# hku-mars/GS-SDF

Hardware: NVIDIA H100
Metric: train_steps_per_s (higher is better)
Workload: dtype f32

## Files before the change

gs-sdf_b200/csrc/sh.cu:

```cuda
#include "common.cuh"

namespace gssdf {

template <int DEG>
__device__ __forceinline__ void sh_bases(float x, float y, float z, float *b) {
    b[0] = 0.2820947917738781f;
    if (DEG < 1) return;
    b[1] = -0.48860251190292f * y; b[2] = 0.48860251190292f * z; b[3] = -0.48860251190292f * x;
    if (DEG < 2) return;
    const float z2 = z * z;
    const float fTmp0B = -1.092548430592079f * z;
    const float fC1 = x * x - y * y, fS1 = 2.f * x * y;
    b[6] = 0.9461746957575601f * z2 - 0.3153915652525201f;
    b[7] = fTmp0B * x; b[5] = fTmp0B * y;
    b[8] = 0.5462742152960395f * fC1; b[4] = 0.5462742152960395f * fS1;
    if (DEG < 3) return;
    const float fTmp0C = -2.285228997322329f * z2 + 0.4570457994644658f;
    const float fTmp1B = 1.445305721320277f * z;
    const float fC2 = x * fC1 - y * fS1, fS2 = x * fS1 + y * fC1;
    b[12] = z * (1.865881662950577f * z2 - 1.119528997770346f);
    b[13] = fTmp0C * x; b[11] = fTmp0C * y;
    b[14] = fTmp1B * fC1; b[10] = fTmp1B * fS1;
    b[15] = -0.5900435899266435f * fC2; b[9] = -0.5900435899266435f * fS2;
    if (DEG < 4) return;
// ... 45 lines not shown
        const float fTmp0D = z * (-4.683325804901025f * z2 + 2.007139630671868f);
        const float fTmp0D_z = 3.f * -4.683325804901025f * z2 + 2.007139630671868f;
        const float fTmp1C = 3.31161143515146f * z2 - 0.47308734787878f;
        const float fTmp1C_z = 2.f * 3.31161143515146f * z;
        const float fTmp2B = -1.770130769779931f * z, fTmp2B_z = -1.770130769779931f;
        const float fC3_x = fC2 + x * fC2_x - y * fS2_x, fC3_y = x * fC2_y - fS2 - y * fS2_y;
        const float fS3_x = fS2 + y * fC2_x + x * fS2_x, fS3_y = x * fS2_y + fC2 + y * fC2_y;
        const float pSH20_z = 1.984313483298443f * (pSH12 + z * pSH12_z) - 1.006230589874905f * pSH6_z;
        vx += 0.6258357354491763f * fS3_x * w[16] + 0.6258357354491763f * fC3_x * w[24] + fTmp2B * fS2_x * w[17] +
              fTmp2B * fC2_x * w[23] + fTmp1C * fS1_x * w[18] + fTmp1C * fC1_x * w[22] + fTmp0D * w[21];
        vy += 0.6258357354491763f * fS3_y * w[16] + 0.6258357354491763f * fC3_y * w[24] + fTmp2B * fS2_y * w[17] +
              fTmp2B * fC2_y * w[23] + fTmp1C * fS1_y * w[18] + fTmp1C * fC1_y * w[22] + fTmp0D * w[19];
        vz += pSH20_z * w[20] + fTmp0D_z * x * w[21] + fTmp0D_z * y * w[19] + fTmp1C_z * fC1 * w[22] +
              fTmp1C_z * fS1 * w[18] + fTmp2B_z * fC2 * w[23] + fTmp2B_z * fS2 * w[17];
    }
}

__device__ __forceinline__ void cam_centre(const float *viewmats, int cid, float c[3]) {
    const float *v = viewmats + 16 * cid;
#pragma unroll
    for (int r = 0; r < 3; ++r) c[r] = -(v[0 + r] * v[3] + v[4 + r] * v[7] + v[8 + r] * v[11]);
}

template <int DEG>
__global__ void __launch_bounds__(256) view_colors_fwd_kernel(const gssdf_view_colors_fwd_args a) {
    constexpr int KU = (DEG + 1) * (DEG + 1);
    const int nnz = a.counts->nnz;
    const int i = blockIdx.x * blockDim.x + threadIdx.x;
    if (i >= nnz) return;
    const int64_t g = a.gaussian_ids[i];
    const int2 rad = reinterpret_cast<const int2 *>(a.radii)[i];
    float out[3] = {0.f, 0.f, 0.f};
    if (rad.x > 0 && rad.y > 0) {
        float cc[3];
        cam_centre(a.viewmats, (int)a.camera_ids[i], cc);
        float dx = a.means[3 * g] - cc[0], dy = a.means[3 * g + 1] - cc[1], dz = a.means[3 * g + 2] - cc[2];
        if (a.mean_offsets) { dx += a.mean_offsets[3 * g]; dy += a.mean_offsets[3 * g + 1]; dz += a.mean_offsets[3 * g + 2]; }
        float x = 0.f, y = 0.f, z = 0.f;
        if (DEG >= 1) {
            const float inorm = rsqrtf(dx * dx + dy * dy + dz * dz);
            x = dx * inorm; y = dy * inorm; z = dz * inorm;
        }
        float b[KU];
        sh_bases<DEG>(x, y, z, b);
        const float *co = a.sh_rest ? a.sh + (size_t)g * 3 : a.sh + (size_t)g * a.K * 3;
        const float *cr = a.sh_rest ? a.sh_rest + (size_t)g * (a.K - 1) * 3 - 3 : co;
#pragma unroll
        for (int k = 0; k < KU; ++k) {
            const float *c = k == 0 ? co : cr + 3 * k;
            out[0] += b[k] * __ldg(c);
            out[1] += b[k] * __ldg(c + 1);
            out[2] += b[k] * __ldg(c + 2);
        }
#pragma unroll
        for (int c = 0; c < 3; ++c) out[c] = fmaxf(out[c] + 0.5f, 0.f);
    }
    a.colors[3 * (int64_t)i] = out[0];
    a.colors[3 * (int64_t)i + 1] = out[1];
    a.colors[3 * (int64_t)i + 2] = out[2];
}

template <int DEG>
__global__ void __launch_bounds__(256) view_colors_bwd_kernel(const gssdf_view_colors_bwd_args a) {
    constexpr int KU = (DEG + 1) * (DEG + 1);
    const int nnz = a.counts->nnz;
    const int i = blockIdx.x * blockDim.x + threadIdx.x;
    if (i >= nnz) return;
    const int2 rad = reinterpret_cast<const int2 *>(a.radii)[i];
    if (!(rad.x > 0 && rad.y > 0)) return;
    const int64_t g = a.gaussian_ids[i];
    float vc[3];
#pragma unroll
    for (int c = 0; c < 3; ++c) {
        const float col = a.colors[3 * (int64_t)i + c];
        vc[c] = col > 0.f ? a.v_colors[3 * (int64_t)i + c] : 0.f;
    }
    float cc[3];
    cam_centre(a.viewmats, (int)a.camera_ids[i], cc);
    float dx = a.means[3 * g] - cc[0], dy = a.means[3 * g + 1] - cc[1], dz = a.means[3 * g + 2] - cc[2];
    if (a.mean_offsets) { dx += a.mean_offsets[3 * g]; dy += a.mean_offsets[3 * g + 1]; dz += a.mean_offsets[3 * g + 2]; }
    float x = 0.f, y = 0.f, z = 0.f, inorm = 1.f;
    if (DEG >= 1) {
// ... 7 lines not shown
    float *vsr = split ? a.v_sh_rest + (size_t)g * (a.K - 1) * 3 - 3 : vsh;
    const float *co = split ? a.sh + (size_t)g * 3 : a.sh + (size_t)g * a.K * 3;
    const float *cr = split ? a.sh_rest + (size_t)g * (a.K - 1) * 3 - 3 : co;
    float w[KU];
#pragma unroll
    for (int k = 0; k < KU; ++k) {
        float *v = k == 0 ? vsh : vsr + 3 * k;
        const float *c = k == 0 ? co : cr + 3 * k;
        atomicAdd(v, b[k] * vc[0]);
        atomicAdd(v + 1, b[k] * vc[1]);
        atomicAdd(v + 2, b[k] * vc[2]);
        w[k] = __ldg(c) * vc[0] + __ldg(c + 1) * vc[1] + __ldg(c + 2) * vc[2];
    }
    if (DEG >= 1 && a.v_means) {
        float vx, vy, vz;
        sh_bases_vjp<DEG>(x, y, z, w, vx, vy, vz);
        const float d = vx * x + vy * y + vz * z;
        atomicAdd(a.v_means + 3 * g, (vx - d * x) * inorm);
        atomicAdd(a.v_means + 3 * g + 1, (vy - d * y) * inorm);
        atomicAdd(a.v_means + 3 * g + 2, (vz - d * z) * inorm);
    }
}

}

using namespace gssdf;

extern "C" int gssdf_view_colors_fwd(const gssdf_view_colors_fwd_args *a, gssdf_stream_t stream) {
    GSSDF_REQUIRE(a != nullptr, GSSDF_EINVAL, "view_colors_fwd: null args");
    if (a->cap == 0 || a->N == 0) return GSSDF_OK;
    GSSDF_REQUIRE(a->sh_degree >= 0 && a->sh_degree <= 4, GSSDF_EINVAL, "view_colors_fwd: sh_degree %d not in [0,4]", a->sh_degree);
    GSSDF_REQUIRE((a->sh_degree + 1) * (a->sh_degree + 1) <= a->K, GSSDF_EINVAL,
                  "view_colors_fwd: Invalid coeffs shape: (deg+1)^2=%d > K=%d", (a->sh_degree + 1) * (a->sh_degree + 1), a->K);
    GSSDF_REQUIRE(a->viewmats && a->means && a->sh && a->counts && a->camera_ids && a->gaussian_ids && a->radii && a->colors,
                  GSSDF_EINVAL, "view_colors_fwd: null pointer");
    cudaStream_t st = (cudaStream_t)stream;
    const int grid = cdiv(a->cap, 256);
    switch (a->sh_degree) {
        case 0: view_colors_fwd_kernel<0><<<grid, 256, 0, st>>>(*a); break;
        case 1: view_colors_fwd_kernel<1><<<grid, 256, 0, st>>>(*a); break;
        case 2: view_colors_fwd_kernel<2><<<grid, 256, 0, st>>>(*a); break;
        case 3: view_colors_fwd_kernel<3><<<grid, 256, 0, st>>>(*a); break;
        default: view_colors_fwd_kernel<4><<<grid, 256, 0, st>>>(*a); break;
    }
    GSSDF_LAUNCH_OK("view_colors_fwd_kernel");
    return GSSDF_OK;
}

extern "C" int gssdf_view_colors_bwd(const gssdf_view_colors_bwd_args *a, gssdf_stream_t stream) {
    GSSDF_REQUIRE(a != nullptr, GSSDF_EINVAL, "view_colors_bwd: null args");
    if (a->cap == 0 || a->N == 0) return GSSDF_OK;
    GSSDF_REQUIRE(a->sh_degree >= 0 && a->sh_degree <= 4, GSSDF_EINVAL, "view_colors_bwd: sh_degree %d not in [0,4]", a->sh_degree);
    GSSDF_REQUIRE((a->sh_degree + 1) * (a->sh_degree + 1) <= a->K, GSSDF_EINVAL, "view_colors_bwd: Invalid coeffs shape");
    GSSDF_REQUIRE(a->viewmats && a->means && a->sh && a->counts && a->camera_ids && a->gaussian_ids && a->radii &&
                      a->colors && a->v_colors && a->v_sh,
                  GSSDF_EINVAL, "view_colors_bwd: null pointer");
    GSSDF_REQUIRE(!a->sh_rest || (a->v_sh_rest && a->K >= 2), GSSDF_EINVAL, "view_colors_bwd: sh_rest needs v_sh_rest and K >= 2");
    cudaStream_t st = (cudaStream_t)stream;
    const int grid = cdiv(a->cap, 256);
    switch (a->sh_degree) {
        case 0: view_colors_bwd_kernel<0><<<grid, 256, 0, st>>>(*a); break;
        case 1: view_colors_bwd_kernel<1><<<grid, 256, 0, st>>>(*a); break;
        case 2: view_colors_bwd_kernel<2><<<grid, 256, 0, st>>>(*a); break;
        case 3: view_colors_bwd_kernel<3><<<grid, 256, 0, st>>>(*a); break;
        default: view_colors_bwd_kernel<4><<<grid, 256, 0, st>>>(*a); break;
    }
    GSSDF_LAUNCH_OK("view_colors_bwd_kernel");
    return GSSDF_OK;
}
```

gs-sdf_b200/gssdf_b200/cabi.py:

```python
import math

import torch

from . import _lib
from ._lib import check, lib, make_args

COUNTS_INTS = 8
NNZ, N_ISECTS, NNZ_OVERFLOW, ISECT_OVERFLOW, MAX_TILE = 0, 1, 2, 3, 4


def _stream():
    return torch.cuda.current_stream().cuda_stream


def _req(t, dtype, name):
    if t is None:
        return None
    if not t.is_cuda:
        raise ValueError(f"gssdf_b200: {name} must be a CUDA tensor")
    if not t.is_contiguous():
        raise ValueError(f"gssdf_b200: {name} must be contiguous")
    if t.dtype != dtype:
        raise ValueError(f"gssdf_b200: {name} must be {dtype}, got {t.dtype}")
    return t
# ... 42 lines not shown
def project2dgs_bwd(means, quats, scales, viewmats, Ks, W, H, cap, counts, camera_ids, gaussian_ids, ray_transforms,
                    randns, v_means2d, v_depths, v_ray_transforms, v_normals, v_samples, v_means, v_quats, v_scales,
                    v_pt_opacities=None, v_opacities=None, mean_offsets=None, raw_params=False, pt_opacities=None):
    a = make_args("gssdf_project2dgs_bwd_args", N=means.shape[0], C=viewmats.shape[0], means=means, quats=quats,
                  scales=scales, viewmats=viewmats, Ks=Ks, image_width=W, image_height=H, cap=cap, counts=counts,
                  camera_ids=camera_ids, gaussian_ids=gaussian_ids, ray_transforms=ray_transforms, randns=randns,
                  v_means2d=v_means2d, v_depths=v_depths, v_ray_transforms=v_ray_transforms, v_normals=v_normals,
                  v_samples=v_samples, v_means=v_means, v_quats=v_quats, v_scales=v_scales,
                  v_pt_opacities=v_pt_opacities, v_opacities=v_opacities, mean_offsets=mean_offsets, raw_params=int(bool(raw_params)),
                  pt_opacities=pt_opacities)
    check(lib().gssdf_project2dgs_bwd(_lib.C.byref(a), _stream()))


def view_colors_fwd(viewmats, means, sh, sh_degree, cap, counts, camera_ids, gaussian_ids, radii, colors, mean_offsets=None,
                    sh_rest=None):
    K = sh.shape[1] + (sh_rest.shape[1] if sh_rest is not None else 0)
    a = make_args("gssdf_view_colors_fwd_args", N=means.shape[0], C=viewmats.shape[0], K=K,
                  sh_degree=sh_degree, viewmats=viewmats, means=means, sh=sh, cap=cap, counts=counts,
                  camera_ids=camera_ids, gaussian_ids=gaussian_ids, radii=radii, colors=colors, mean_offsets=mean_offsets,
                  sh_rest=sh_rest)
    check(lib().gssdf_view_colors_fwd(_lib.C.byref(a), _stream()))


def view_colors_bwd(viewmats, means, sh, sh_degree, cap, counts, camera_ids, gaussian_ids, radii, colors, v_colors,
                    v_sh, v_means, mean_offsets=None, sh_rest=None, v_sh_rest=None):
    K = sh.shape[1] + (sh_rest.shape[1] if sh_rest is not None else 0)
    a = make_args("gssdf_view_colors_bwd_args", N=means.shape[0], C=viewmats.shape[0], K=K,
                  sh_degree=sh_degree, viewmats=viewmats, means=means, sh=sh, cap=cap, counts=counts,
                  camera_ids=camera_ids, gaussian_ids=gaussian_ids, radii=radii, colors=colors, v_colors=v_colors,
                  v_sh=v_sh, v_means=v_means, mean_offsets=mean_offsets, sh_rest=sh_rest, v_sh_rest=v_sh_rest)
    check(lib().gssdf_view_colors_bwd(_lib.C.byref(a), _stream()))


def tile_encode(Cn, W, H, tile_size, cap, counts, means2d, radii, depths, camera_ids, isect_cap, tiles_per_gauss,
                isect_ids, flatten_ids, offsets, ws, conics=None):
    need = lib().gssdf_tile_encode_workspace_bytes(Cn, W, H, tile_size, isect_cap)
    w = ws.get(need)
    a = make_args("gssdf_tile_encode_args", C=Cn, image_width=W, image_height=H, tile_size=tile_size, cap=cap,
                  counts=counts, means2d=means2d, radii=radii, depths=depths, camera_ids=camera_ids, isect_cap=isect_cap,
                  tiles_per_gauss=tiles_per_gauss, isect_ids=isect_ids, flatten_ids=flatten_ids, offsets=offsets,
                  workspace=w, workspace_bytes=w.numel(), conics=conics)
    check(lib().gssdf_tile_encode(_lib.C.byref(a), _stream()))


def splat_conics(cap, W, H, counts, ray_transforms, opacities, conics):
    a = make_args("gssdf_splat_conics_args", cap=cap, image_width=W, image_height=H, counts=counts, ray_transforms=ray_transforms,
                  opacities=opacities, conics=conics)
    check(lib().gssdf_splat_conics(_lib.C.byref(a), _stream()))


def raster2dgs_fwd(Cn, W, H, tile_size, channels, cap, counts, means2d, ray_transforms, colors, opacities, normals,
                   backgrounds, offsets, flatten_ids, out, ws, prof=None, isect_cap=None):
    isect_cap = int(flatten_ids.shape[0]) if isect_cap is None else int(isect_cap)
    need = lib().gssdf_raster2dgs_workspace_bytes(Cn, W, H, cap, _lib.C.c_int64(isect_cap))
# ... 385 lines not shown
```

gs-sdf_b200/gssdf_b200/render.py:

```python
import contextlib
import math

import torch

from . import cabi


def check_photometric(who, bck_color, mask, H, W, device):
    if isinstance(bck_color, bool) or bck_color not in (0, 1, 2):
        raise ValueError(f"{who}: bck_color must be 0 (black), 1 (white) or 2 (random), got {bck_color!r}")
    if mask is None:
        return
    if not isinstance(mask, torch.Tensor) or mask.dtype not in (torch.bool, torch.uint8):
        raise ValueError(f"{who}: mask must be a bool or uint8 tensor, got {getattr(mask, 'dtype', type(mask))}")
    if H is not None and tuple(mask.shape) not in ((H, W), (H, W, 1), (H, W, 3)):
        raise ValueError(f"{who}: mask must be [H,W], [H,W,1] or [H,W,3] with H={H}, W={W}, got {tuple(mask.shape)}")
    dev = torch.device(device)
    if not mask.is_cuda or dev.type != "cuda" or (dev.index is not None and mask.device.index != dev.index):
        raise ValueError(f"{who}: mask must be on {dev}, got {mask.device}")


def check_depth_type(who, depth_type):
    if isinstance(depth_type, bool) or not isinstance(depth_type, int):
        raise ValueError(f"{who}: depth_type must be an int (0: expected depth, otherwise the median depth), got {depth_type!r}")
# ... 52 lines not shown
        self.r["visibilities"] = e(cap, 1)
        self.g = dict(v_means2d=None, v_ray_transforms=e(cap, 3, 3), v_colors=e(cap, 3), v_opacities=e(cap),
                      v_normals=e(cap, 3), v_densify=e(cap, 2))
        sizes = [N * 3, N * 4, N * 3, N, N * K * 3]
        self.flat_grad = torch.zeros(sum(sizes), **f32)
        o = [0]
        for s in sizes:
            o.append(o[-1] + s)
        fg = self.flat_grad
        self.v_means, self.v_quats = fg[o[0]:o[1]].view(N, 3), fg[o[1]:o[2]].view(N, 4)
        self.v_scales, self.v_opac, self.v_sh = fg[o[2]:o[3]].view(N, 3), fg[o[3]:o[4]], fg[o[4]:o[5]].view(N, K, 3)
        self.loss = torch.zeros(1, **f32)
        self.ws = cabi.Workspace(device)
        self.raster_ws = cabi.Workspace(device)
        self.loss_ws = cabi.Workspace(device)
        L, i64 = cabi.lib(), cabi._lib.C.c_int64
        self.raster_ws.get(max(L.gssdf_raster2dgs_bwd_workspace_bytes(C, w, h, cap, i64(self.isect_cap)) for w, h in self.frame_sizes))
        if frame_sizes:
            self.ws.get(max(max(L.gssdf_tile_encode_workspace_bytes(C, w, h, tile_size, i64(self.isect_cap)),
                                L.gssdf_project2dgs_workspace_bytes(N, C)) for w, h in self.frame_sizes))
            self.loss_ws.get(max(L.gssdf_dssim_workspace_bytes(C, w, h) for w, h in self.frame_sizes))
        self.prof_fwd = self.prof_bwd = None
        self.stage_events = None

    def set_frame(self, W, H):
        W, H = int(W), int(H)
        if (W, H) == (self.W, self.H):
            return
        tw, th = math.ceil(W / self.tile), math.ceil(H / self.tile)
        if W < 1 or H < 1 or W * H > self.max_pixels or tw * th > self.max_tiles:
            raise ValueError(f"SplatRenderer.set_frame: a {W}x{H} frame does not fit storage for {self.max_pixels} pixels and "
                             f"{self.max_tiles} tiles (frame_sizes)")
        C = self.C
        self.W, self.H, self.tw, self.th = W, H, tw, th
        for grp, key, ch, _, _ in _PIXEL_BUFFERS:
            st = self._pix[(grp, key)]
            v = st[:C * H * W * (ch or 1)].view((C, H, W, ch) if ch else (C, H, W))
            if grp is None:
                setattr(self, key, v)
            else:
                getattr(self, grp)[key] = v
        self.offsets = self._offsets_store[:C * th * tw].view(C, th, tw)

    def _zero_pixels(self, grp, key):
        self._pix[(grp, key)].zero_()

    def _mark(self, name):
        if self.stage_events is not None:
            ev = torch.cuda.Event(enable_timing=True)
            ev.record()
            self.stage_events.append((name, ev))

    def forward(self, means, quats, scales, opacities, sh, viewmats, Ks, randns=None, raw=None, bck_color=0, bg=None):
        C, W, H, cap = self.C, self.W, self.H, self.cap
        off, rest = (raw["offsets"], raw["sh_rest"]) if raw else (None, None)
        cabi.project2dgs_fwd(means, quats, scales, viewmats, Ks, W, H, self.near, self.far, 0.0, randns, cap, self.p,
                             self.counts, self.ws, opacities=opacities, mean_offsets=off, raw_params=raw is not None)
        self._mark("projection_fwd")
        if raw and raw.get("sh_catch_up") is not None:
            raw["sh_catch_up"]()
        cabi.view_colors_fwd(viewmats, means, sh, self.sh_degree, cap, self.counts, self.p["camera_ids"],
                             self.p["gaussian_ids"], self.p["radii"], self.colors, mean_offsets=off, sh_rest=rest)
        self._mark("sh_fwd")
        conics = None
        if self.presort_cull:
            cabi.splat_conics(cap, W, H, self.counts, self.p["ray_transforms"], self.p["pt_opacities"], self.conics)
            conics = self.conics
        cabi.tile_encode(C, W, H, self.tile, cap, self.counts, self.p["means2d"], self.p["radii"], self.p["depths"],
                         self.p["camera_ids"], self.isect_cap, None, None, self.flatten_ids, self.offsets, self.ws, conics=conics)
        self._mark("tile_encode")
        cabi.raster2dgs_fwd(C, W, H, self.tile, 3, cap, self.counts, self.p["means2d"], self.p["ray_transforms"], self.colors,
                            self.p["pt_opacities"], self.p["normals"], None, self.offsets, self.flatten_ids, self.r, self.raster_ws,
                            prof=self.prof_fwd, isect_cap=self.isect_cap)
        self._mark("raster_fwd")
        if bck_color:
            cabi.render_post_bg_fwd(C, W, H, viewmats, self.r["render_colors"], self.r["render_depths"], self.r["render_alphas"],
                                    self.r["render_normals"], self.out_colors, self.out_normals, bck_color, bg)
        else:
            cabi.render_post_fwd(C, W, H, viewmats, self.r["render_colors"], self.r["render_depths"], self.r["render_alphas"],
                                 self.r["render_normals"], self.out_colors, self.out_normals)
        self._mark("post_fwd")
        return self.out_colors, self.out_normals

    def backward(self, means, quats, scales, opacities, sh, viewmats, Ks, gt, randns=None, w_rgb=1.0, w_depth=0.1, v_samples=None,
                 zero_grads=True, raw=None, w_dssim=0.0, w_normal=0.0, w_isotropic=0.0, before_projection_bwd=None, projection_bwd=True,
# ... 31 lines not shown
        if not (w_normal > 0 and median_depth) and getattr(self, "_v_median_dirty", False):
            self._zero_pixels("v_r", "median")
            self._v_median_dirty = False
        if w_isotropic > 0:
            cabi.isotropic_loss(self.N, cap, self.counts, self.p["gaussian_ids"], scales, raw is not None, w_isotropic, self.loss,
                                self.v_scales)
        if bck_color:
            cabi.render_post_bg_bwd(C, W, H, viewmats, self.r["render_depths"], self.r["render_alphas"], self.v_out_colors,
                                    self.v_out_normals, None, self.v_r["colors"], self.v_r["depths"], self.v_r["alphas"],
                                    self.v_r["normals"], bck_color, bg)
        else:
            cabi.render_post_bwd(C, W, H, viewmats, self.r["render_depths"], self.r["render_alphas"], self.v_out_colors,
                                 self.v_out_normals, None, self.v_r["colors"], self.v_r["depths"], self.v_r["alphas"],
                                 self.v_r["normals"])
        self._mark("losses+post_bwd")
        cabi.raster2dgs_bwd(C, W, H, self.tile, 3, cap, self.counts, self.p["means2d"], self.p["ray_transforms"], self.colors,
                            self.p["pt_opacities"], self.p["normals"], None, self.offsets, self.flatten_ids,
                            self.r["render_alphas"], None, self.r["last_ids"], self.r["median_ids"],
                            self.v_r["colors"], self.v_r["depths"], self.v_r["alphas"], self.v_r["normals"],
                            self.v_r["median"], self.g, self.raster_ws, prof=self.prof_bwd, isect_cap=self.isect_cap, reuse_fwd=True)
        self._mark("raster_bwd")
        cabi.view_colors_bwd(viewmats, means, sh, self.sh_degree, cap, self.counts, self.p["camera_ids"],
                             self.p["gaussian_ids"], self.p["radii"], self.colors, self.g["v_colors"], v_sh, self.v_means,
                             mean_offsets=off, sh_rest=rest, v_sh_rest=v_rest)
        self._mark("sh_bwd")
        if not projection_bwd:
            return self.loss
        if before_projection_bwd is not None:
            before_projection_bwd()
        cabi.project2dgs_bwd(means, quats, scales, viewmats, Ks, W, H, cap, self.counts, self.p["camera_ids"],
                             self.p["gaussian_ids"], self.p["ray_transforms"], randns, None, None, self.g["v_ray_transforms"],
                             self.g["v_normals"], v_samples, self.v_means, self.v_quats, self.v_scales,
                             v_pt_opacities=self.g["v_opacities"], v_opacities=self.v_opac, mean_offsets=off,
                             raw_params=raw is not None, pt_opacities=self.p["pt_opacities"])
        self._mark("projection_bwd")
        return self.loss

    def step(self, scene, viewmats, Ks, gt, randns=None):
        raw = scene.get("raw")
        self.forward(scene["means"], scene["quats"], scene["scales"], scene["opacities"], scene["sh"], viewmats, Ks, randns, raw=raw)
        return self.backward(scene["means"], scene["quats"], scene["scales"], scene["opacities"], scene["sh"], viewmats, Ks, gt,
                             randns, raw=raw)

    KERNELS_PER_STEP = 21

    def read_counts(self):
        c = self.counts.cpu().tolist()
# ... 70 lines not shown
        if mask is not None:
            self.mask = expand_mask(mask, self.R.H, self.R.W)

    def view_frame(self, W, H):
        self.R.set_frame(W, H)
        if self._bg_store is not None:
            self.bg = self._bg_store[:3 * self.R.H * self.R.W].view(1, self.R.H, self.R.W, 3)

    @contextlib.contextmanager
    def sdf_stage(self):
        if not (self.overlap and self.overlap_ray_stage):
            yield
            return
        side = self._side_stream()
        side.wait_stream(torch.cuda.current_stream())
        with torch.cuda.stream(side):
            yield

    def _side_stream(self):
        if self._side is None:
            self._side = torch.cuda.Stream(device=self.dev, priority=self.sdf_stream_priority)
        return self._side

    KERNELS_PER_STEP = SplatRenderer.KERNELS_PER_STEP + 10

    def _rebind_splat_grads(self, n_splat):
        R, N, K = self.R, self.R.N, self.R.K
        R.flat_grad = self.flat_grad[:n_splat]
        o = [0, N * 3, N * 7, N * 10, N * 11, N * 11 + N * K * 3]
        fg = R.flat_grad
        R.v_means, R.v_quats, R.v_scales = fg[o[0]:o[1]].view(N, 3), fg[o[1]:o[2]].view(N, 4), fg[o[2]:o[3]].view(N, 3)
        R.v_opac, R.v_sh = fg[o[3]:o[4]], fg[o[4]:o[5]].view(N, K, 3)

    def refresh_table(self, table_f32):
        cabi.sdf_table_to_half(table_f32, self.table_half)

    def set_octree(self, octree):
        self.octree = octree
        self.valid_mask = torch.zeros(self.R.cap, dtype=torch.uint8, device=self.dev) if octree is not None else None

    def _coupling_compact(self, net, samples, n_live, on_sdf_grads_ready):
        R, cap = self.R, self.R.cap
        cabi.sdf_gate_compact(cap, samples, self.gate_idx, self.gate_x, self.n_gate, self.gate_ws, visibilities=R.r["visibilities"],
                              visible_thr=self.vis_thr, valid_mask=self.valid_mask, weights=R.p["sample_weights"], w_out=self.gate_w,
                              n_live=n_live)
        if self.eik_mode == 1 and self.delta_dev is not None:
            if self.align_w > 0:
# ... 179 lines not shown
        self._exp_avg = t

    @property
    def exp_avg_sq(self):
        self.flush_sh()
        return self._exp_avg_sq

    @exp_avg_sq.setter
    def exp_avg_sq(self, t):
        self._exp_avg_sq = t

    def flush_sh(self):
        if not self._sh_stale:
            return
        self._sh_stale = False
        cabi.adam_step(self._params, self.flat_grad, self._exp_avg, self._exp_avg_sq, self._sh_groups(), self.t_sh,
                       replay=self.sh_replay, replay_only=True)

    def _sh_groups(self):
        o, w, n = self.seg_off, self.seg_w, self.N_live
        return [(o[4], n * w[4], self.lr[4], False, w[4]), (o[5], n * w[5], self.lr[5], False, w[5])]

    def _sh_catch_up(self):
        if self.t_sh > 0:
            cabi.adam_step(self._params, self.flat_grad, self._exp_avg, self._exp_avg_sq, self._sh_groups(), self.t_sh,
                           replay=self.sh_replay, row_ids=self.R.p["gaussian_ids"], row_count=self.R.counts, row_cap=self.R.cap,
                           replay_only=True)

    def stamp_sh_current(self):
        self.sh_last.fill_(self.t_sh)
        self._sh_stale = False

    def set_live(self, n_live):
        assert 0 <= n_live <= self.N_cap
        if self.N_live is not None and int(n_live) != self.N_live:
            self.flush_sh()
            self.stamp_sh_current()
        self.N_live = n = int(n_live)
        o, w, pv, K = self.seg_off, self.seg_w, self._params, self.R.K
        v = lambda s_, *shape: pv[o[s_]:o[s_] + n * w[s_]].view(n, *shape)
        self.anchors = self.anchors_buf[:n]
        catch_up = self._sh_catch_up if self.lazy_sh else None
        self.scene = dict(means=self.anchors, quats=v(1, 4), scales=v(2, 3), opacities=pv[o[3]:o[3] + n], sh=v(4, 1, 3),
                          raw=dict(offsets=v(0, 3), sh_rest=v(5, K - 1, 3) if K > 1 else None, sh_catch_up=catch_up))
        self.splat_groups = [(o[i], n * w[i], self.lr[i], False, w[i] if (self.lazy_sh and i >= 4) else 0)
                             for i in range(6) if w[i] > 0 and n > 0]
        self.splat_group_is_sh = [i >= 4 for i in range(6) if w[i] > 0 and n > 0]
        t0 = self.t0
        self.sdf_groups = [(t0, self.n_table, self.sdf_lr, True), (t0 + self.n_table, self.n_mlp, self.sdf_lr, False)]
        self.table, self.mlp = pv[t0:t0 + self.n_table], pv[t0 + self.n_table:]
# ... 103 lines not shown
```

include/gssdf_b200.h:

```cpp
#ifndef GSSDF_B200_H
#define GSSDF_B200_H

#include <stddef.h>
#include <stdint.h>

#ifdef __cplusplus
extern "C" {
#endif

typedef struct CUstream_st *gssdf_stream_t;

enum {
    GSSDF_OK = 0,
    GSSDF_EINVAL = -1,
    GSSDF_ECUDA = -2,
    GSSDF_EUNSUPPORTED = -3,
    GSSDF_ENOMEM = -4
};

const char *gssdf_last_error(void);
const char *gssdf_version(void);
#define GSSDF_ABI_REVISION 18
int32_t gssdf_abi_revision(void);

// ... 90 lines not shown
    const int32_t *radii;
    float *colors;
    const float *mean_offsets;
    const float *sh_rest;
} gssdf_view_colors_fwd_args;
int gssdf_view_colors_fwd(const gssdf_view_colors_fwd_args *a, gssdf_stream_t stream);

typedef struct gssdf_view_colors_bwd_args {
    int32_t N, C, K, sh_degree;
    const float *viewmats, *means, *sh;
    int32_t cap;
    const gssdf_counts *counts;
    const int64_t *camera_ids, *gaussian_ids;
    const int32_t *radii;
    const float *colors;
    const float *v_colors;
    float *v_sh;
    float *v_means;
    const float *mean_offsets;
    const float *sh_rest;
    float *v_sh_rest;
} gssdf_view_colors_bwd_args;
int gssdf_view_colors_bwd(const gssdf_view_colors_bwd_args *a, gssdf_stream_t stream);

typedef struct gssdf_tile_encode_args {
    int32_t C;
    int32_t image_width, image_height, tile_size;
    int32_t cap;
    gssdf_counts *counts;
    const float *means2d;
    const int32_t *radii;
    const float *depths;
    const int64_t *camera_ids;
    int64_t isect_cap;
    int32_t *tiles_per_gauss;
    int64_t *isect_ids;
    int32_t *flatten_ids;
    int32_t *offsets;
    void *workspace;
    size_t workspace_bytes;
    const float *conics;
} gssdf_tile_encode_args;
size_t gssdf_tile_encode_workspace_bytes(int32_t C, int32_t image_width, int32_t image_height,
                                         int32_t tile_size, int64_t isect_cap);
typedef struct gssdf_splat_conics_args {
    int32_t cap;
// ... 334 lines not shown
} gssdf_adam_group;

typedef struct gssdf_adam_args {
    float *params;
    float *grads;
    float *exp_avg, *exp_avg_sq;
    int32_t n_groups;
    gssdf_adam_group groups[GSSDF_ADAM_MAX_GROUPS];
    int32_t step;
    float beta1, beta2, eps;
    float grad_scale;
    int32_t zero_grads;
    void *table_half;
    const gssdf_sdf_net *net;
    void *mlp_packed;
    const gssdf_adam_replay *replay;
    const int64_t *row_ids;
    const gssdf_counts *row_count;
    int32_t row_cap;
    int32_t replay_only;
} gssdf_adam_args;
int gssdf_adam_step(const gssdf_adam_args *a, gssdf_stream_t stream);
int gssdf_adam_step_clocks(const gssdf_adam_args *a, const int32_t *group_steps, gssdf_stream_t stream);

#define GSSDF_ROWS_MAX_SEGMENTS 8
typedef struct gssdf_row_segment {
    int64_t offset;
    int32_t width, pad_;
} gssdf_row_segment;
typedef struct gssdf_rows_args {
    int32_t n_segments;
    int32_t zero_source;
    gssdf_row_segment segments[GSSDF_ROWS_MAX_SEGMENTS];
    int64_t cap_rows;
    const int32_t *n_rows;
    const int64_t *row_ids;
    float *flat;
    float *packed;
} gssdf_rows_args;
int gssdf_rows_pack(const gssdf_rows_args *a, gssdf_stream_t stream);
int gssdf_rows_unpack_add(const gssdf_rows_args *a, gssdf_stream_t stream);

typedef struct gssdf_densify_update_args {
    int32_t N, cap;
    const gssdf_counts *counts;
    const int64_t *gaussian_ids;
// ... 397 lines not shown
```

Before: 209.2.

## Fuse lazy SH Adam catch-up into view-color forward and reuse rows in backward

Folds the replay-only Adam catch-up for visible SH rows into the view-color forward kernel. Each CTA stages 64 rows in shared memory, replays the missed optimizer steps and writes the caught-up coefficients to a compact rows buffer. The backward pass reads that buffer and does coalesced per-CTA staging, with non-atomic read-modify-write gradient accumulation into v_sh, which relies on single-camera visible rows being distinct. This removes one kernel launch and the scattered re-reads of SH rows, at the cost of a C==1 restriction, an extra cap×3K buffer, and no longer writing caught-up params back to the parameter store in this path.

```diff
diff --git a/gs-sdf_b200/csrc/sh.cu b/gs-sdf_b200/csrc/sh.cu
--- a/gs-sdf_b200/csrc/sh.cu
+++ b/gs-sdf_b200/csrc/sh.cu
@@ -1,3 +1,4 @@
+#include "adam.cuh"
 #include "common.cuh"
 
 namespace gssdf {
@@ -91,42 +92,108 @@
     for (int r = 0; r < 3; ++r) c[r] = -(v[0 + r] * v[3] + v[4 + r] * v[7] + v[8 + r] * v[11]);
 }
 
+template <int DEG, class Coef>
+__device__ __forceinline__ void view_color(const gssdf_view_colors_fwd_args &a, int i, int64_t g, Coef coef, float out[3]) {
+    constexpr int KU = (DEG + 1) * (DEG + 1);
+    out[0] = out[1] = out[2] = 0.f;
+    const int2 rad = reinterpret_cast<const int2 *>(a.radii)[i];
+    if (!(rad.x > 0 && rad.y > 0)) return;
+    float cc[3];
+    cam_centre(a.viewmats, (int)a.camera_ids[i], cc);
+    float dx = a.means[3 * g] - cc[0], dy = a.means[3 * g + 1] - cc[1], dz = a.means[3 * g + 2] - cc[2];
+    if (a.mean_offsets) { dx += a.mean_offsets[3 * g]; dy += a.mean_offsets[3 * g + 1]; dz += a.mean_offsets[3 * g + 2]; }
+    float x = 0.f, y = 0.f, z = 0.f;
+    if (DEG >= 1) {
+        const float inorm = rsqrtf(dx * dx + dy * dy + dz * dz);
+        x = dx * inorm; y = dy * inorm; z = dz * inorm;
+    }
+    float b[KU];
+    sh_bases<DEG>(x, y, z, b);
+#pragma unroll
+    for (int k = 0; k < KU; ++k) {
+        out[0] += b[k] * coef(k, 0);
+        out[1] += b[k] * coef(k, 1);
+        out[2] += b[k] * coef(k, 2);
+    }
+#pragma unroll
+    for (int c = 0; c < 3; ++c) out[c] = fmaxf(out[c] + 0.5f, 0.f);
+}
+
 template <int DEG>
 __global__ void __launch_bounds__(256) view_colors_fwd_kernel(const gssdf_view_colors_fwd_args a) {
-    constexpr int KU = (DEG + 1) * (DEG + 1);
     const int nnz = a.counts->nnz;
     const int i = blockIdx.x * blockDim.x + threadIdx.x;
     if (i >= nnz) return;
     const int64_t g = a.gaussian_ids[i];
-    const int2 rad = reinterpret_cast<const int2 *>(a.radii)[i];
-    float out[3] = {0.f, 0.f, 0.f};
-    if (rad.x > 0 && rad.y > 0) {
-        float cc[3];
-        cam_centre(a.viewmats, (int)a.camera_ids[i], cc);
-        float dx = a.means[3 * g] - cc[0], dy = a.means[3 * g + 1] - cc[1], dz = a.means[3 * g + 2] - cc[2];
-        if (a.mean_offsets) { dx += a.mean_offsets[3 * g]; dy += a.mean_offsets[3 * g + 1]; dz += a.mean_offsets[3 * g + 2]; }
-        float x = 0.f, y = 0.f, z = 0.f;
-        if (DEG >= 1) {
-            const float inorm = rsqrtf(dx * dx + dy * dy + dz * dz);
-            x = dx * inorm; y = dy * inorm; z = dz * inorm;
-        }
-        float b[KU];
-        sh_bases<DEG>(x, y, z, b);
-        const float *co = a.sh_rest ? a.sh + (size_t)g * 3 : a.sh + (size_t)g * a.K * 3;
-        const float *cr = a.sh_rest ? a.sh_rest + (size_t)g * (a.K - 1) * 3 - 3 : co;
-#pragma unroll
-        for (int k = 0; k < KU; ++k) {
-            const float *c = k == 0 ? co : cr + 3 * k;
-            out[0] += b[k] * __ldg(c);
-            out[1] += b[k] * __ldg(c + 1);
-            out[2] += b[k] * __ldg(c + 2);
-        }
-#pragma unroll
-        for (int c = 0; c < 3; ++c) out[c] = fmaxf(out[c] + 0.5f, 0.f);
-    }
+    const float *co = a.sh_rest ? a.sh + (size_t)g * 3 : a.sh + (size_t)g * a.K * 3;
+    const float *cr = a.sh_rest ? a.sh_rest + (size_t)g * (a.K - 1) * 3 - 3 : co;
+    float out[3];
+    view_color<DEG>(a, i, g, [&](int k, int c) { return __ldg((k == 0 ? co : cr + 3 * k) + c); }, out);
     a.colors[3 * (int64_t)i] = out[0];
     a.colors[3 * (int64_t)i + 1] = out[1];
     a.colors[3 * (int64_t)i + 2] = out[2];
+}
+
+struct ShRows {
+    const float *p, *m, *v;
+    float *rows;
+    int64_t off0, off1;
+    int32_t w0, w, stride, step;
+};
+
+constexpr int kRowsPerCta = 64, kRowThreads = 256, kRowBatch = 4;
+
+template <int DEG>
+__global__ void __launch_bounds__(kRowThreads) view_colors_fwd_lazy_kernel(const gssdf_view_colors_fwd_args a, const ShRows L,
+                                                                           const gssdf_adam_replay r) {
+    extern __shared__ float s_p[];
+    __shared__ int64_t s_g[kRowsPerCta];
+    __shared__ int32_t s_last[kRowsPerCta];
+    const int nnz = min(a.counts->nnz, a.cap);
+    const int i0 = blockIdx.x * kRowsPerCta, tid = threadIdx.x;
+    if (i0 >= nnz) return;
+    const int nr = min(kRowsPerCta, nnz - i0);
+    if (tid < nr) {
+        const int64_t g = a.gaussian_ids[i0 + tid];
+        s_g[tid] = g;
+        s_last[tid] = r.last[g];
+    }
+    __syncthreads();
+    const int total = nr * L.w;
+    for (int e0 = tid; e0 < total; e0 += kRowThreads * kRowBatch) {
+        int64_t j[kRowBatch];
+        float p[kRowBatch], m[kRowBatch], v[kRowBatch];
+        int from[kRowBatch], gk[kRowBatch], si[kRowBatch];
+#pragma unroll
+        for (int u = 0; u < kRowBatch; ++u) {
+            const int e = e0 + u * kRowThreads;
+            si[u] = -1;
+            if (e >= total) continue;
+            const int kr = e / L.w, c = e - kr * L.w;
+            gk[u] = c >= L.w0 ? 1 : 0;
+            j[u] = gk[u] ? L.off1 + s_g[kr] * (L.w - L.w0) + (c - L.w0) : L.off0 + s_g[kr] * L.w0 + c;
+            si[u] = kr * L.stride + c;
+            from[u] = s_last[kr];
+            p[u] = __ldg(L.p + j[u]);
+            if (from[u] < L.step) { m[u] = __ldg(L.m + j[u]); v[u] = __ldg(L.v + j[u]); }
+        }
+#pragma unroll
+        for (int u = 0; u < kRowBatch; ++u) {
+            if (si[u] < 0) continue;
+            if (from[u] < L.step) adam_replay(p[u], m[u], v[u], from[u], L.step, r, gk[u]);
+            s_p[si[u]] = p[u];
+            L.rows[(int64_t)i0 * L.w + e0 + u * kRowThreads] = p[u];
+        }
+    }
+    __syncthreads();
+    if (tid >= nr) return;
+    const float *row = s_p + tid * L.stride;
+    float out[3];
+    view_color<DEG>(a, i0 + tid, s_g[tid], [&](int k, int c) { return row[3 * k + c]; }, out);
+    const int64_t i = i0 + tid;
+    a.colors[3 * i] = out[0];
+    a.colors[3 * i + 1] = out[1];
+    a.colors[3 * i + 2] = out[2];
 }
 
 template <int DEG>
@@ -180,18 +247,122 @@
     }
 }
 
+__device__ __forceinline__ float add_ftz(float a, float b) {
+    float s;
+    asm("add.rn.ftz.f32 %0, %1, %2;" : "=f"(s) : "f"(a), "f"(b));
+    return s;
+}
+
+template <int DEG>
+__global__ void __launch_bounds__(kRowThreads) view_colors_bwd_rows_kernel(const gssdf_view_colors_bwd_args a, const float *rows) {
+    constexpr int KU = (DEG + 1) * (DEG + 1), WU = 3 * KU, STRIDE = WU | 1;
+    __shared__ float s_row[kRowsPerCta * STRIDE];
+    __shared__ int64_t s_g[kRowsPerCta];
+    const int nnz = min(a.counts->nnz, a.cap);
+    const int i0 = blockIdx.x * kRowsPerCta, tid = threadIdx.x;
+    if (i0 >= nnz) return;
+    const int nr = min(kRowsPerCta, nnz - i0);
+    const bool split = a.sh_rest != nullptr;
+    const int wr = split ? 3 * (a.K - 1) : 3 * a.K;
+    if (tid < nr) {
+        const int2 rad = reinterpret_cast<const int2 *>(a.radii)[i0 + tid];
+        s_g[tid] = (rad.x > 0 && rad.y > 0) ? a.gaussian_ids[i0 + tid] : -1;
+    }
+    __syncthreads();
+    for (int e0 = tid; e0 < nr * WU; e0 += kRowThreads * kRowBatch) {
+        float x[kRowBatch];
+#pragma unroll
+        for (int u = 0; u < kRowBatch; ++u) {
+            const int e = e0 + u * kRowThreads, kr = e / WU, c = e - kr * WU;
+            const int64_t g = e < nr * WU ? s_g[kr] : -1;
+            if (g < 0) continue;
+            if (rows) x[u] = __ldg(rows + (int64_t)(i0 + kr) * (3 * a.K) + c);
+            else x[u] = split ? (c < 3 ? __ldg(a.sh + g * 3 + c) : __ldg(a.sh_rest + g * wr + (c - 3))) : __ldg(a.sh + g * wr + c);
+        }
+#pragma unroll
+        for (int u = 0; u < kRowBatch; ++u) {
+            const int e = e0 + u * kRowThreads, kr = e / WU, c = e - kr * WU;
+            if (e < nr * WU && s_g[kr] >= 0) s_row[kr * STRIDE + c] = x[u];
+        }
+    }
+    __syncthreads();
+    const int64_t g = tid < nr ? s_g[tid] : -1;
+    if (g >= 0) {
+        const int i = i0 + tid;
+        float vc[3];
+#pragma unroll
+        for (int c = 0; c < 3; ++c) {
+            const float col = a.colors[3 * (int64_t)i + c];
+            vc[c] = col > 0.f ? a.v_colors[3 * (int64_t)i + c] : 0.f;
+        }
+        float cc[3];
+        cam_centre(a.viewmats, (int)a.camera_ids[i], cc);
+        float dx = a.means[3 * g] - cc[0], dy = a.means[3 * g + 1] - cc[1], dz = a.means[3 * g + 2] - cc[2];
+        if (a.mean_offsets) { dx += a.mean_offsets[3 * g]; dy += a.mean_offsets[3 * g + 1]; dz += a.mean_offsets[3 * g + 2]; }
+        float x = 0.f, y = 0.f, z = 0.f, inorm = 1.f;
+        if (DEG >= 1) {
+            inorm = rsqrtf(dx * dx + dy * dy + dz * dz);
+            x = dx * inorm; y = dy * inorm; z = dz * inorm;
+        }
+        float b[KU];
+        sh_bases<DEG>(x, y, z, b);
+        float *row = s_row + tid * STRIDE;
+        float w[KU];
+#pragma unroll
+        for (int k = 0; k < KU; ++k) {
+            float *c = row + 3 * k;
+            w[k] = c[0] * vc[0] + c[1] * vc[1] + c[2] * vc[2];
+            c[0] = b[k] * vc[0];
+            c[1] = b[k] * vc[1];
+            c[2] = b[k] * vc[2];
+        }
+        if (DEG >= 1 && a.v_means) {
+            float vx, vy, vz;
+            sh_bases_vjp<DEG>(x, y, z, w, vx, vy, vz);
+            const float d = vx * x + vy * y + vz * z;
+            atomicAdd(a.v_means + 3 * g, (vx - d * x) * inorm);
+            atomicAdd(a.v_means + 3 * g + 1, (vy - d * y) * inorm);
+            atomicAdd(a.v_means + 3 * g + 2, (vz - d * z) * inorm);
+        }
+    }
+    __syncthreads();
+    for (int e0 = tid; e0 < nr * WU; e0 += kRowThreads * kRowBatch) {
+        float *v[kRowBatch];
+        float x[kRowBatch];
+#pragma unroll
+        for (int u = 0; u < kRowBatch; ++u) {
+            const int e = e0 + u * kRowThreads, kr = e / WU, c = e - kr * WU;
+            const int64_t gg = e < nr * WU ? s_g[kr] : -1;
+            v[u] = nullptr;
+            if (gg < 0) continue;
+            v[u] = split ? (c < 3 ? a.v_sh + gg * 3 + c : a.v_sh_rest + gg * wr + (c - 3)) : a.v_sh + gg * wr + c;
+            x[u] = *v[u];
+        }
+#pragma unroll
+        for (int u = 0; u < kRowBatch; ++u) {
+            const int e = e0 + u * kRowThreads, kr = e / WU, c = e - kr * WU;
+            if (v[u]) *v[u] = add_ftz(x[u], s_row[kr * STRIDE + c]);
+        }
+    }
+}
+
 }
 
 using namespace gssdf;
+
+static int view_colors_fwd_check(const gssdf_view_colors_fwd_args *a, const char *who) {
+    GSSDF_REQUIRE(a->sh_degree >= 0 && a->sh_degree <= 4, GSSDF_EINVAL, "%s: sh_degree %d not in [0,4]", who, a->sh_degree);
+    GSSDF_REQUIRE((a->sh_degree + 1) * (a->sh_degree + 1) <= a->K, GSSDF_EINVAL,
+                  "%s: Invalid coeffs shape: (deg+1)^2=%d > K=%d", who, (a->sh_degree + 1) * (a->sh_degree + 1), a->K);
+    GSSDF_REQUIRE(a->viewmats && a->means && a->sh && a->counts && a->camera_ids && a->gaussian_ids && a->radii && a->colors,
+                  GSSDF_EINVAL, "%s: null pointer", who);
+    return GSSDF_OK;
+}
 
 extern "C" int gssdf_view_colors_fwd(const gssdf_view_colors_fwd_args *a, gssdf_stream_t stream) {
     GSSDF_REQUIRE(a != nullptr, GSSDF_EINVAL, "view_colors_fwd: null args");
     if (a->cap == 0 || a->N == 0) return GSSDF_OK;
-    GSSDF_REQUIRE(a->sh_degree >= 0 && a->sh_degree <= 4, GSSDF_EINVAL, "view_colors_fwd: sh_degree %d not in [0,4]", a->sh_degree);
-    GSSDF_REQUIRE((a->sh_degree + 1) * (a->sh_degree + 1) <= a->K, GSSDF_EINVAL,
-                  "view_colors_fwd: Invalid coeffs shape: (deg+1)^2=%d > K=%d", (a->sh_degree + 1) * (a->sh_degree + 1), a->K);
-    GSSDF_REQUIRE(a->viewmats && a->means && a->sh && a->counts && a->camera_ids && a->gaussian_ids && a->radii && a->colors,
-                  GSSDF_EINVAL, "view_colors_fwd: null pointer");
+    if (const int rc = view_colors_fwd_check(a, "view_colors_fwd")) return rc;
     cudaStream_t st = (cudaStream_t)stream;
     const int grid = cdiv(a->cap, 256);
     switch (a->sh_degree) {
@@ -205,7 +376,50 @@
     return GSSDF_OK;
 }
 
-extern "C" int gssdf_view_colors_bwd(const gssdf_view_colors_bwd_args *a, gssdf_stream_t stream) {
+extern "C" int gssdf_view_colors_fwd_lazy(const gssdf_view_colors_fwd_args *a, const gssdf_adam_args *u, float *rows,
+                                          gssdf_stream_t stream) {
+    GSSDF_REQUIRE(a != nullptr && u != nullptr, GSSDF_EINVAL, "view_colors_fwd_lazy: null args");
+    if (a->cap == 0 || a->N == 0) return GSSDF_OK;
+    if (const int rc = view_colors_fwd_check(a, "view_colors_fwd_lazy")) return rc;
+    GSSDF_REQUIRE(a->C == 1, GSSDF_EINVAL, "view_colors_fwd_lazy: C = %d, needs 1 camera (distinct visible rows)", a->C);
+    GSSDF_REQUIRE(rows && u->params && u->exp_avg && u->exp_avg_sq && u->replay && u->replay->last, GSSDF_EINVAL,
+                  "view_colors_fwd_lazy: null buffer");
+    GSSDF_REQUIRE(u->replay_only && u->row_ids == a->gaussian_ids && u->row_count == a->counts && u->row_cap == a->cap, GSSDF_EINVAL,
+                  "view_colors_fwd_lazy: the catch-up must be replay-only over the visible rows (row_ids = gaussian_ids, row_count = "
+                  "counts, row_cap = cap)");
+    GSSDF_REQUIRE(u->step >= 1 && u->replay->step == u->step, GSSDF_EINVAL, "view_colors_fwd_lazy: step %d, replay at step %d", u->step,
+                  u->replay->step);
+    GSSDF_REQUIRE(u->replay->beta1 == u->beta1 && u->replay->beta2 == u->beta2 && u->replay->eps == u->eps, GSSDF_EINVAL,
+                  "view_colors_fwd_lazy: replay constants differ from the step's");
+    const bool split = a->sh_rest != nullptr;
+    GSSDF_REQUIRE(u->n_groups == (split ? 2 : 1), GSSDF_EINVAL, "view_colors_fwd_lazy: %d groups, the %s layout has %d", u->n_groups,
+                  split ? "split" : "unsplit", split ? 2 : 1);
+    const float *row_base[2] = {a->sh, a->sh_rest};
+    const int32_t width[2] = {split ? 3 : 3 * a->K, 3 * (a->K - 1)};
+    for (int k = 0; k < u->n_groups; ++k) {
+        const gssdf_adam_group &g = u->groups[k];
+        GSSDF_REQUIRE(g.row_width == width[k] && g.count == (int64_t)a->N * width[k] && g.offset >= 0 && !g.half_shadow &&
+                          u->params + g.offset == row_base[k],
+                      GSSDF_EINVAL, "view_colors_fwd_lazy: group %d is not the SH rows the forward reads", k);
+    }
+    const ShRows L{u->params, u->exp_avg, u->exp_avg_sq, rows, u->groups[0].offset, split ? u->groups[1].offset : 0, width[0], 3 * a->K,
+                   (3 * a->K) | 1, u->step};
+    const size_t smem = (size_t)kRowsPerCta * L.stride * sizeof(float);
+    GSSDF_REQUIRE(smem <= 48 * 1024, GSSDF_EINVAL, "view_colors_fwd_lazy: K = %d rows do not fit shared memory", a->K);
+    cudaStream_t st = (cudaStream_t)stream;
+    const int grid = cdiv(a->cap, kRowsPerCta);
+    switch (a->sh_degree) {
+        case 0: view_colors_fwd_lazy_kernel<0><<<grid, kRowThreads, smem, st>>>(*a, L, *u->replay); break;
+        case 1: view_colors_fwd_lazy_kernel<1><<<grid, kRowThreads, smem, st>>>(*a, L, *u->replay); break;
+        case 2: view_colors_fwd_lazy_kernel<2><<<grid, kRowThreads, smem, st>>>(*a, L, *u->replay); break;
+        case 3: view_colors_fwd_lazy_kernel<3><<<grid, kRowThreads, smem, st>>>(*a, L, *u->replay); break;
+        default: view_colors_fwd_lazy_kernel<4><<<grid, kRowThreads, smem, st>>>(*a, L, *u->replay); break;
+    }
+    GSSDF_LAUNCH_OK("view_colors_fwd_lazy_kernel");
+    return GSSDF_OK;
+}
+
+static int view_colors_bwd_launch(const gssdf_view_colors_bwd_args *a, const float *rows, gssdf_stream_t stream) {
     GSSDF_REQUIRE(a != nullptr, GSSDF_EINVAL, "view_colors_bwd: null args");
     if (a->cap == 0 || a->N == 0) return GSSDF_OK;
     GSSDF_REQUIRE(a->sh_degree >= 0 && a->sh_degree <= 4, GSSDF_EINVAL, "view_colors_bwd: sh_degree %d not in [0,4]", a->sh_degree);
@@ -214,7 +428,20 @@
                       a->colors && a->v_colors && a->v_sh,
                   GSSDF_EINVAL, "view_colors_bwd: null pointer");
     GSSDF_REQUIRE(!a->sh_rest || (a->v_sh_rest && a->K >= 2), GSSDF_EINVAL, "view_colors_bwd: sh_rest needs v_sh_rest and K >= 2");
+    GSSDF_REQUIRE(!rows || a->C == 1, GSSDF_EINVAL, "view_colors_bwd_rows: C = %d, needs 1 camera", a->C);
     cudaStream_t st = (cudaStream_t)stream;
+    if (a->C == 1) {
+        const int grid = cdiv(a->cap, kRowsPerCta);
+        switch (a->sh_degree) {
+            case 0: view_colors_bwd_rows_kernel<0><<<grid, kRowThreads, 0, st>>>(*a, rows); break;
+            case 1: view_colors_bwd_rows_kernel<1><<<grid, kRowThreads, 0, st>>>(*a, rows); break;
+            case 2: view_colors_bwd_rows_kernel<2><<<grid, kRowThreads, 0, st>>>(*a, rows); break;
+            case 3: view_colors_bwd_rows_kernel<3><<<grid, kRowThreads, 0, st>>>(*a, rows); break;
+            default: view_colors_bwd_rows_kernel<4><<<grid, kRowThreads, 0, st>>>(*a, rows); break;
+        }
+        GSSDF_LAUNCH_OK("view_colors_bwd_rows_kernel");
+        return GSSDF_OK;
+    }
     const int grid = cdiv(a->cap, 256);
     switch (a->sh_degree) {
         case 0: view_colors_bwd_kernel<0><<<grid, 256, 0, st>>>(*a); break;
@@ -226,3 +453,12 @@
     GSSDF_LAUNCH_OK("view_colors_bwd_kernel");
     return GSSDF_OK;
 }
+
+extern "C" int gssdf_view_colors_bwd(const gssdf_view_colors_bwd_args *a, gssdf_stream_t stream) {
+    return view_colors_bwd_launch(a, nullptr, stream);
+}
+
+extern "C" int gssdf_view_colors_bwd_rows(const gssdf_view_colors_bwd_args *a, const float *rows, gssdf_stream_t stream) {
+    GSSDF_REQUIRE(rows != nullptr, GSSDF_EINVAL, "view_colors_bwd_rows: null rows");
+    return view_colors_bwd_launch(a, rows, stream);
+}
diff --git a/gs-sdf_b200/gssdf_b200/cabi.py b/gs-sdf_b200/gssdf_b200/cabi.py
--- a/gs-sdf_b200/gssdf_b200/cabi.py
+++ b/gs-sdf_b200/gssdf_b200/cabi.py
@@ -88,14 +88,28 @@
     check(lib().gssdf_view_colors_fwd(_lib.C.byref(a), _stream()))
 
 
+def view_colors_fwd_lazy(viewmats, means, sh, sh_degree, cap, counts, camera_ids, gaussian_ids, radii, colors, catch_up, rows,
+                         mean_offsets=None, sh_rest=None):
+    K = sh.shape[1] + (sh_rest.shape[1] if sh_rest is not None else 0)
+    a = make_args("gssdf_view_colors_fwd_args", N=means.shape[0], C=viewmats.shape[0], K=K,
+                  sh_degree=sh_degree, viewmats=viewmats, means=means, sh=sh, cap=cap, counts=counts,
+                  camera_ids=camera_ids, gaussian_ids=gaussian_ids, radii=radii, colors=colors, mean_offsets=mean_offsets,
+                  sh_rest=sh_rest)
+    u = _adam_args(**catch_up)
+    check(lib().gssdf_view_colors_fwd_lazy(_lib.C.byref(a), _lib.C.byref(u), _req(rows, torch.float32, "rows").data_ptr(), _stream()))
+
+
 def view_colors_bwd(viewmats, means, sh, sh_degree, cap, counts, camera_ids, gaussian_ids, radii, colors, v_colors,
-                    v_sh, v_means, mean_offsets=None, sh_rest=None, v_sh_rest=None):
+                    v_sh, v_means, mean_offsets=None, sh_rest=None, v_sh_rest=None, rows=None):
     K = sh.shape[1] + (sh_rest.shape[1] if sh_rest is not None else 0)
     a = make_args("gssdf_view_colors_bwd_args", N=means.shape[0], C=viewmats.shape[0], K=K,
                   sh_degree=sh_degree, viewmats=viewmats, means=means, sh=sh, cap=cap, counts=counts,
                   camera_ids=camera_ids, gaussian_ids=gaussian_ids, radii=radii, colors=colors, v_colors=v_colors,
                   v_sh=v_sh, v_means=v_means, mean_offsets=mean_offsets, sh_rest=sh_rest, v_sh_rest=v_sh_rest)
-    check(lib().gssdf_view_colors_bwd(_lib.C.byref(a), _stream()))
+    if rows is None:
+        check(lib().gssdf_view_colors_bwd(_lib.C.byref(a), _stream()))
+    else:
+        check(lib().gssdf_view_colors_bwd_rows(_lib.C.byref(a), _req(rows, torch.float32, "rows").data_ptr(), _stream()))
 
 
 def tile_encode(Cn, W, H, tile_size, cap, counts, means2d, radii, depths, camera_ids, isect_cap, tiles_per_gauss,
diff --git a/gs-sdf_b200/gssdf_b200/render.py b/gs-sdf_b200/gssdf_b200/render.py
--- a/gs-sdf_b200/gssdf_b200/render.py
+++ b/gs-sdf_b200/gssdf_b200/render.py
@@ -98,6 +98,7 @@
             self.loss_ws.get(max(L.gssdf_dssim_workspace_bytes(C, w, h) for w, h in self.frame_sizes))
         self.prof_fwd = self.prof_bwd = None
         self.stage_events = None
+        self.sh_rows, self._sh_rows_live = None, False
 
     def set_frame(self, W, H):
         W, H = int(W), int(H)
@@ -133,10 +134,18 @@
         cabi.project2dgs_fwd(means, quats, scales, viewmats, Ks, W, H, self.near, self.far, 0.0, randns, cap, self.p,
                              self.counts, self.ws, opacities=opacities, mean_offsets=off, raw_params=raw is not None)
         self._mark("projection_fwd")
-        if raw and raw.get("sh_catch_up") is not None:
-            raw["sh_catch_up"]()
-        cabi.view_colors_fwd(viewmats, means, sh, self.sh_degree, cap, self.counts, self.p["camera_ids"],
-                             self.p["gaussian_ids"], self.p["radii"], self.colors, mean_offsets=off, sh_rest=rest)
+        catch_up = raw["sh_catch_up"]() if raw and raw.get("sh_catch_up") is not None else None
+        self._sh_rows_live = catch_up is not None and C == 1
+        if self._sh_rows_live:
+            if self.sh_rows is None:
+                self.sh_rows = torch.empty(cap, 3 * self.K, dtype=torch.float32, device=means.device)
+            cabi.view_colors_fwd_lazy(viewmats, means, sh, self.sh_degree, cap, self.counts, self.p["camera_ids"], self.p["gaussian_ids"],
+                                      self.p["radii"], self.colors, catch_up, self.sh_rows, mean_offsets=off, sh_rest=rest)
+        else:
+            if catch_up is not None:
+                cabi.adam_step(**catch_up)
+            cabi.view_colors_fwd(viewmats, means, sh, self.sh_degree, cap, self.counts, self.p["camera_ids"],
+                                 self.p["gaussian_ids"], self.p["radii"], self.colors, mean_offsets=off, sh_rest=rest)
         self._mark("sh_fwd")
         conics = None
         if self.presort_cull:
@@ -214,7 +223,7 @@
         self._mark("raster_bwd")
         cabi.view_colors_bwd(viewmats, means, sh, self.sh_degree, cap, self.counts, self.p["camera_ids"],
                              self.p["gaussian_ids"], self.p["radii"], self.colors, self.g["v_colors"], v_sh, self.v_means,
-                             mean_offsets=off, sh_rest=rest, v_sh_rest=v_rest)
+                             mean_offsets=off, sh_rest=rest, v_sh_rest=v_rest, rows=self.sh_rows if self._sh_rows_live else None)
         self._mark("sh_bwd")
         if not projection_bwd:
             return self.loss
@@ -331,7 +340,7 @@
             self._side = torch.cuda.Stream(device=self.dev, priority=self.sdf_stream_priority)
         return self._side
 
-    KERNELS_PER_STEP = SplatRenderer.KERNELS_PER_STEP + 10
+    KERNELS_PER_STEP = SplatRenderer.KERNELS_PER_STEP + 9
 
     def _rebind_splat_grads(self, n_splat):
         R, N, K = self.R, self.R.N, self.R.K
@@ -557,10 +566,11 @@
         return [(o[4], n * w[4], self.lr[4], False, w[4]), (o[5], n * w[5], self.lr[5], False, w[5])]
 
     def _sh_catch_up(self):
-        if self.t_sh > 0:
-            cabi.adam_step(self._params, self.flat_grad, self._exp_avg, self._exp_avg_sq, self._sh_groups(), self.t_sh,
-                           replay=self.sh_replay, row_ids=self.R.p["gaussian_ids"], row_count=self.R.counts, row_cap=self.R.cap,
-                           replay_only=True)
+        if self.t_sh == 0:
+            return None
+        return dict(params=self._params, grads=self.flat_grad, exp_avg=self._exp_avg, exp_avg_sq=self._exp_avg_sq,
+                    groups=self._sh_groups(), step=self.t_sh, replay=self.sh_replay, row_ids=self.R.p["gaussian_ids"],
+                    row_count=self.R.counts, row_cap=self.R.cap, replay_only=True)
 
     def stamp_sh_current(self):
         self.sh_last.fill_(self.t_sh)
diff --git a/include/gssdf_b200.h b/include/gssdf_b200.h
--- a/include/gssdf_b200.h
+++ b/include/gssdf_b200.h
@@ -136,6 +136,7 @@
     float *v_sh_rest;
 } gssdf_view_colors_bwd_args;
 int gssdf_view_colors_bwd(const gssdf_view_colors_bwd_args *a, gssdf_stream_t stream);
+int gssdf_view_colors_bwd_rows(const gssdf_view_colors_bwd_args *a, const float *rows, gssdf_stream_t stream);
 
 typedef struct gssdf_tile_encode_args {
     int32_t C;
@@ -516,6 +517,7 @@
 } gssdf_adam_args;
 int gssdf_adam_step(const gssdf_adam_args *a, gssdf_stream_t stream);
 int gssdf_adam_step_clocks(const gssdf_adam_args *a, const int32_t *group_steps, gssdf_stream_t stream);
+int gssdf_view_colors_fwd_lazy(const gssdf_view_colors_fwd_args *a, const gssdf_adam_args *u, float *rows, gssdf_stream_t stream);
 
 #define GSSDF_ROWS_MAX_SEGMENTS 8
 typedef struct gssdf_row_segment {
```

New measurement: 214.6, median of 6. 1.03x the previous value.
